# brocksam/pycollo

Measured on AMD Instinct MI355X. Metric: NLP-callback evals/sec (g + jac_g + hess), higher is better.
Workload: dtype f64; 1 GPU; hypersensitive, 1 phase, 2000 mesh sections x 6 Lobatto nodes = 10001 collocation nodes; num_x=20003, num_c=10001, nnz_jac=140003, nnz_hess=20002, tiles=167, threads_per_block=64, waves_per_tile=4, launches_per_eval=1, lds_bytes_per_workgroup=24144, launch_thread_cpu=16, pin_survived_hip_init=False

## Files before the change

__graft_entry__.py:

```python
from __future__ import annotations

import os
import subprocess
import sys

ROOT = os.path.dirname(os.path.abspath(__file__))
if ROOT not in sys.path:
    sys.path.insert(0, ROOT)

CSRC = os.path.join(ROOT, "pycollo_amd", "csrc")
LIB = os.path.join(ROOT, "pycollo_amd", "libpycollo_amd.so")


def _run(cmd):
    res = subprocess.run(cmd, capture_output=True, text=True)
    if res.returncode != 0:
        raise RuntimeError(f"{' '.join(cmd)} failed:\n{res.stdout[-2000:]}\n{res.stderr[-4000:]}")


def _stale(target, sources):
    if not os.path.exists(target):
        return True
    t = os.path.getmtime(target)
    return any(os.path.getmtime(s) > t for s in sources)


def build_library(force: bool = False) -> str:
    srcs = [os.path.join(CSRC, f) for f in ("pc_engine.hip", "pc_kkt.hip", "pc_host.hpp", "pc_ipm.hpp", "pc_kkt_cr.hpp", "pc_kkt_shape.hpp", "pc_eval_shape.hpp", "pc_eval_launch.hpp", "pc_pattern.hpp", "pc_desc.hpp", "pc_args.h", "pc_deriv.hpp", "pc_deriv_check.hpp",
                                           "pc_solution_plan.hpp", "pc_costate_plan.hpp", "pc_propagate_plan.hpp",
                                           "pc_solution_host.hpp")]
    srcs.append(os.path.join(ROOT, "include", "pycollo_amd.h"))
    if force or _stale(LIB, srcs):
        hipcc = "/opt/rocm/bin/hipcc" if os.path.exists("/opt/rocm/bin/hipcc") else "hipcc"
        _run([hipcc, "--offload-arch=gfx950", "-O2", "-ffp-contract=off", "-fPIC", "-shared", "-std=c++17", "-o", LIB + ".tmp",
              os.path.join(CSRC, "pc_engine.hip"), os.path.join(CSRC, "pc_kkt.hip")])
        os.replace(LIB + ".tmp", LIB)
    return LIB


PREBUILD = [
    ("brachistochrone", {}, (0,)), ("brachistochrone", {}, (4,)),
    ("hypersensitive", {}, (0,)), ("hypersensitive", {}, (6,)), ("hypersensitive", {}, (5,)), ("hypersensitive", {}, (4,)),
    ("hypersensitive", {}, (2,)), ("hypersensitive", {}, (8,)), ("hypersensitive", {}, (3,)),
    ("hypersensitive", {"fixed_control": 0.0}, (0,)),
    ("cart_pole", {}, (0,)), ("cart_pole", {}, (4,)), ("cart_pole", {}, (5,)),
    ("shuttle", {}, (0,)), ("shuttle", {}, (4,)), ("shuttle", {}, (5,)), ("shuttle", {}, (6,)),
    ("double_pendulum", {}, (0,)), ("double_pendulum", {}, (4,)),
    ("two_phase_transfer", {}, (0, 0)), ("two_phase_transfer", {}, (3, 4)), ("two_phase_transfer", {}, (4, 5)),
    ("two_phase_transfer", {}, (2, 2)), ("two_phase_transfer", {}, (3, 3)), ("two_phase_transfer", {}, (4, 4)),
    ("time_coupled_transfer", {}, (0, 0)), ("time_coupled_transfer", {}, (4, 4)),
    ("time_coupled_transfer", {}, (3, 3)), ("time_coupled_transfer", {}, (3, 4)),
    ("delta_iii", {}, (0, 0, 0, 0)), ("delta_iii", {}, (4, 4, 4, 4)), ("delta_iii", {}, (5, 5, 5, 5)), ("delta_iii", {}, (8, 8, 8, 8)),
    ("free_flying_robot", {}, (0,)), ("free_flying_robot", {}, (4,)), ("free_flying_robot", {}, (5,)),
    ("tumour_anti_angiogenesis", {}, (0,)), ("tumour_anti_angiogenesis", {}, (4,)), ("tumour_anti_angiogenesis", {}, (6,)),
    ("space_station", {}, (0,)), ("space_station", {}, (4,)),
    ("sliding_mass", {"num_phases": 1}, (0,)), ("sliding_mass", {"num_phases": 1}, (4,)),
    ("sliding_mass", {"num_phases": 2}, (0, 0)), ("sliding_mass", {"num_phases": 2}, (4, 4)),
    ("sliding_mass", {"num_phases": 3}, (0, 0, 0)), ("sliding_mass", {"num_phases": 3}, (4, 4, 4)),
    ("sliding_mass", {"num_phases": 4}, (0, 0, 0, 0)), ("sliding_mass", {"num_phases": 4}, (4, 4, 4, 4)),
    ("function_family", {"family": "powers"}, (0,)), ("function_family", {"family": "powers"}, (4,)),
    ("function_family", {"family": "trig"}, (0,)), ("function_family", {"family": "trig"}, (4,)),
    ("function_family", {"family": "special"}, (0,)), ("function_family", {"family": "special"}, (4,)),
    ("function_family", {"family": "kinks"}, (0,)), ("function_family", {"family": "kinks"}, (4,)),
]
PREBUILD_MIXED = [
    ("hypersensitive", {}, (4, 6)), ("cart_pole", {}, (4, 6)), ("shuttle", {}, (4, 6)), ("double_pendulum", {}, (4, 6)),
    ("two_phase_transfer", {}, (4, 6)), ("time_coupled_transfer", {}, (4, 6)), ("delta_iii", {}, (4, 6)),
    ("hypersensitive", {}, (6,)), ("two_phase_transfer", {}, (4,)), ("time_coupled_transfer", {}, (4,)), ("delta_iii", {}, (5,)),
# ... 104 lines not shown
```

pycollo_amd/codegen.py:

```python
from __future__ import annotations

import hashlib
import os
import shutil
import subprocess

import sympy as sym
from sympy.printing.c import C99CodePrinter

from .model import Model, PhaseModel, PointModel

CSRC = os.path.join(os.path.dirname(os.path.abspath(__file__)), "csrc")
CACHE = os.path.join(os.path.dirname(os.path.abspath(__file__)), "_cache")
ARCH = "gfx950"


class _Printer(C99CodePrinter):

    def _print_Pow(self, expr):
        base, exp = expr.base, expr.exp
        b = self.parenthesize(base, 200)
        if exp.is_Integer:
            n = int(exp)
            if n == 0:
# ... 285 lines not shown
    if heavy_cap is None:
        heavy_cap = _heavy_cap_enabled()
    heavy_any = any(is_heavy(pm) for pm in model.phases)
    parts = [f"// generated by pycollo_amd.codegen for model '{model.name}' digest {model.digest} -- do not edit",
             '#include "pc_kernels.hpp"',
             '#include "pc_solution.hpp"',
             "",
             POWI_PRELUDE,
             "namespace gen {"]
    for pm in model.phases:
        parts.append(_phase_struct(pm, model))
    parts.append(_point_struct(model.point))
    parts.append("}  // namespace gen\n")
    parts.append("namespace gen {")
    parts.append("struct Tail {   // finishes one evaluation: cross-tile sums of every phase and the endpoint block")
    parts.append("  // RES: block 0 of a resident-tail bulk launch (values of other workgroups arrive as granules)")
    parts.append("  template <bool RES = false, bool BIG = false>")
    parts.append("  __device__ static __forceinline__ void run(const PcTailArgs& a, const PcTailLead* ld = nullptr, int arg_off = 0,")
    parts.append("                                             int tb = 0, int ntb = 1) {")
    parts.append("    extern __shared__ double pc_tail_smem[];")
    parts.append("    const pc::TailLds L = pc::tail_lds<Point>(a, pc_tail_smem);")
    first = model.phases[0].index
    parts.append("    if constexpr (RES) {")
    parts.append("      pc::KernargWarm warm;")
    parts.append("      warm.issue<(int)sizeof(PcTailArgs)>(arg_off);   // every line of the tail's argument block, at once")
    parts.append("      pc::tail_point_load<Point, true>(a, L);")
    parts.append("      pc::tail_begin(a, L);")
    parts.append("      warm.settle();")
    parts.append("      pc::tail_point_eval<Point>(a, L, tb, ntb);   // the endpoint rows are out before the first tile's sums arrive")
    parts.append("      if (tb > 0) { pc::tail_point_publish<Point>(a, L, tb, ntb); return; }   // helper block: its parts only")
    for pm in model.phases:
        parts.append(f"      pc::tail_phase<Phase{pm.index}, true>(a, {pm.index}, L);")
    parts.append("      pc::tail_point_collect<Point>(a, L, ntb);")
    parts.append("      pc::tail_point_apply<Point, true>(a, L);")
    parts.append("      pc::tail_end(a, L);")
    parts.append("    } else {")
    parts.append(f"      pc::TailPhaseRegs<Phase{first}> r0;   // the first phase's loads go out before anything else")
    parts.append(f"      pc::tail_phase_issue<Phase{first}, false, BIG>(a, {first}, r0, ld);")
    parts.append("      __builtin_amdgcn_sched_barrier(0);")
    parts.append("      pc::tail_point_load<Point, false>(a, L);")
    parts.append("      pc::tail_begin(a, L);")
    parts.append("      pc::tail_point_eval<Point>(a, L);")
    parts.append(f"      pc::tail_phase_finish<Phase{first}>(a, {first}, r0, L);")
    for pm in model.phases[1:]:
        parts.append(f"      pc::tail_phase<Phase{pm.index}, false, BIG>(a, {pm.index}, L);")
    parts.append("      pc::tail_point_apply<Point, false>(a, L);")
    parts.append("      pc::tail_end(a, L);")
    parts.append("    }")
    parts.append("  }")
    parts.append("};")
    parts.append("}  // namespace gen\n")
    occ = _occupancy_attr()
    lead_sig = ('const double* xz, const double* lamd, const double* qa, const double* sec_h, int N, int K, '
                'int tile_begin, int n_blocks, int wa, int wb')
    parts.append("#ifndef PC_PART\n#define PC_PART -1\n#endif")
    parts.append("#if PC_PART <= 0")
    for pm in model.phases:
        hv = _heavy_attr(is_heavy(pm), heavy_cap)
        parts.append(f'extern "C" __global__ void __launch_bounds__(256) {occ}{hv}pc_bulk_p{pm.index}({lead_sig}, PcPhaseArgs a) {{')
        if mixed[pm.index] and len(model.phases) == 1:
            parts.append('  const PcPhaseArgs& ka = pc::kernarg_phase_args();   // (a itself is not named: see there)')
            parts.append('  const int blk = pc::xcd_major((int)blockIdx.x, n_blocks);')
            parts.append(f'  pc::bulk_mix<gen::Phase{pm.index}, false, 0, 0>({seq(pm)}, ka.tile_rec + blk, ka, false, 0, blk);')
        else:
            parts.append('  const PcLead ld{xz, lamd, qa, sec_h, N, K, tile_begin, n_blocks, wa, wb};')
            parts.append(f'  pc::bulk<gen::Phase{pm.index}, {int(orders[pm.index])}>(a, false, 0, -1, &ld);')
        parts.append('}')
    parts.append("#endif")
    if len(model.phases) == 1:
        pm = model.phases[0]
# ... 320 lines not shown
```

pycollo_amd/csrc/pc_kernels.hpp:

```cpp
#pragma once

#include <hip/hip_runtime.h>
#include <type_traits>
#include <utility>

#include "pc_args.h"

namespace pc {

template <int I>
using ic = std::integral_constant<int, I>;

template <int B, int E, class F>
__device__ __forceinline__ void static_for(F&& f) {
  if constexpr (B < E) {
    f(ic<B>{});
    static_for<B + 1, E>(f);
  }
}

#ifndef PC_SPLIT_MIN
#define PC_SPLIT_MIN 90
#endif

// ... 374 lines not shown

#ifndef PC_XCD_SWIZZLE
#define PC_XCD_SWIZZLE 1
#endif
__device__ __forceinline__ int xcd_major(int b, int nb) {
#if PC_XCD_SWIZZLE
  constexpr int NX = 8;
  const int q = nb / NX, r = nb % NX, x = b % NX, j = b / NX;
  return x * q + (x < r ? x : r) + j;
#else
  (void)nb;
  return b;
#endif
}

#ifdef PC_STAMPS
#ifndef PC_STAMPS_WAVES
#define PC_STAMPS_WAVES 16384
#endif
extern "C" __device__ unsigned long long pc_stamps[PC_STAMPS_WAVES * 24];
#define PC_STAMP(i)                                                                                         \
  do {                                                                                                      \
    if ((threadIdx.x & 63) == 0 && pc_stamp_slot < PC_STAMPS_WAVES)                                         \
      pc_stamps[(size_t)pc_stamp_slot * 24 + (i)] = (i) == 9 ? __builtin_amdgcn_s_memrealtime() : __builtin_amdgcn_s_memtime(); \
  } while (0)
#else
#define PC_STAMP(i) do { } while (0)
#endif

template <class M, int UN, bool RES = false, int WN = 0, int WIDX = 0, bool MIX = false>
__device__ __forceinline__ void bulk(const PcPhaseArgs& KA, bool MULTI = false, int first_block = 0, int block = -1,
                                     const PcLead* LD = nullptr, const double* mx = nullptr, const double* mlam = nullptr,
                                     double* mc = nullptr, double* mG = nullptr, double* mH = nullptr, int mflags = 0,
                                     unsigned mepoch = 0, int r_k0 = 0, int r_nsec = 0, int r_n0 = 0, int r_nprev = 0,
                                     int r_qaprev = 0, long long r_E0 = 0, double r_wprev = 0.0) {
  using St = S<M>;
  constexpr int NY = St::NY, NZ = St::NZ, NQ = St::NQ, NP = St::NP, NS = St::NS, NT = St::NT;
  constexpr int NFN = St::NFN, NV = St::NV, NJ = St::NJ, NH = St::NH, NFS = St::NFS, NRED = St::NRED;
  constexpr bool PURE = MIX && UN > 0;
  BulkIn<St> A;
  if (LD) {
    const int wa = LD->wa, wb = LD->wb;
    A.xz = LD->xz; A.lamd = LD->lamd; A.qa = LD->qa; A.sec_h = LD->sec_h; A.N = LD->N; A.K = LD->K;
    A.tile_begin = LD->tile_begin; A.n_blocks = LD->n_blocks;
    A.flags = pc_wa_flags(wa); A.wpt = pc_wa_wpt(wa); A.block_threads = pc_wa_block_threads(wa); A.spt = pc_wa_spt(wa);
    A.qa0 = pc_wb_qa_off(wb); A.qwabs = pc_wb_qw_abs(wb);
  } else {
    A.x = MULTI ? mx : KA.x; A.lam = MULTI ? mlam : KA.lam; A.x_off = KA.x_off; A.c_off = KA.c_off; A.N = KA.N; A.K = KA.K;
    A.xz = A.x + A.x_off; A.lamd = A.lam + A.c_off; A.qa = KA.qa; A.sec_h = KA.sec_h;
    A.tile_begin = KA.tile_begin; A.spt = KA.spt; A.n_blocks = KA.n_blocks;
// ... 214 lines not shown
    goff = A.goff;
    hoff = A.hoff;
  } else {
    sc = s_tab;
    goff = reinterpret_cast<const int64_t*>(s_tab + St::NSCAL);
    hoff = goff + NFN;
  }
  const bool owns = active && (t < T || last_tile);
  double F[NFN > 0 ? NFN : 1], Jv[NJ > 0 ? NJ : 1], Hv[NH > 0 ? NH : 1], mu[NFN > 0 ? NFN : 1];
  double red[NRED > 0 ? NRED : 1];
  static_for<0, NRED>([&](auto r_) { red[decltype(r_)::value] = 0.0; });
  if (active) {
    static_for<0, NS>([&](auto l_) {
      constexpr int l = decltype(l_)::value;
      constexpr int kind = M::wk(l), idx = M::wi(l);
      v[NZ + l] = A.x[kind == 0 ? A.s_off + idx : A.x_off + (int64_t)NZ * N + (kind == 1 ? idx : NQ + idx)];
    });
  }
  double lam_p[NP > 0 ? NP : 1], lam_q[NQ > 0 ? NQ : 1];
  if (owns && wantH && hess_replica) {
    static_for<0, NP>([&](auto m_) { lam_p[decltype(m_)::value] = A.lam[A.c_path_off + (int64_t) decltype(m_)::value * N + node]; });
    static_for<0, NQ>([&](auto m_) { lam_q[decltype(m_)::value] = A.lam[A.c_int_off + decltype(m_)::value]; });
  }

  const int r_off = (UN == 0 && tid < 2 * (PC_MAX_ORDER + 1)) ? reinterpret_cast<const int32_t*>(&KA.qa_off[0])[tid] : 0;
  if (!early_aux) aux_loads();
  if constexpr (UN == 0) {
    r_qa = tid < A.qa_total ? A.qa[tid] : 0.0;
    r_qw = tid < A.qw_total ? A.qw[tid] : 0.0;
  }
  pin_second_group();
  if (!uni) {
    for (int i = tid; i <= nsec; i += TB) {
      s_s[i] = A.sec_s[kp + i];
      s_E[i] = A.sec_E[kp + i];
    }
  }
  if (UN == 0 && tid < 2 * (PC_MAX_ORDER + 1)) s_off[tid] = r_off;
  if constexpr (UN > 0) {
    if (tid < QA_N) s_qa[tid] = r_qa;
    if (tid < UN) s_qw[tid] = r_qw;
  } else {
    if (tid < A.qa_total) s_qa[tid] = r_qa;
    if (tid < A.qw_total) s_qw[tid] = r_qw;
  }
  if (tid < nsec) s_h[tid] = r_h;
// ... 197 lines not shown
      const double sr = wave_sum(red[r]);
      if (lane == 0) s_red[r * 16 + wave] = sr;
    });
    if constexpr (RES) {
      lds_barrier();
      if (tid < NRED) {
        double sr = 0.0;
        for (int ww = 0; ww < nw; ++ww) sr += s_red[tid * 16 + ww];
        publish_granules(A.gran + 2 * ((int64_t)tile * NRED + tid), A.epoch, sr);
      }
    }
  }
  };
  constexpr bool SPLIT = ((NJ + NH >= PC_SPLIT_MIN) || M::HEAVY) && St::NWT == 0;
  constexpr bool RED_EARLY = RES && NS == 0 && NRED > 0;
  double mult[NFN > 0 ? NFN : 1];
  if (active) {
    static_for<0, NFN>([&](auto r_) {
      constexpr int r = decltype(r_)::value;
      mult[r] = (r >= NY && r < NY + NP) ? mu[r] : stretch * mu[r];
    });
  }
  const int n_own = T + (last_tile ? 1 : 0);
  const bool edge0 = (node == 0), edgeN = (node == N - 1);
  constexpr int NEDGE = St::NHZZ + 2 * NZ + NS * NZ;
  auto edge_store = [&](auto site_, double* dstp, double val) {
    constexpr int site = decltype(site_)::value;
    constexpr bool f0 = M::efl(site) != 0, fN = M::efl(NEDGE + site) != 0;
    if constexpr (RES && (f0 || fN)) {
      constexpr int r0 = PC_CE(St::erank(site)), rN = PC_CE(St::erank(NEDGE + site));
      if (edge0 ? f0 : fN) {
        publish_granules(A.erec + 2 * (int64_t)(A.erec0 + (edge0 ? r0 : rN)), A.epoch, val);
        return;
      }
    }
    *dstp = val;
  };
  auto hess_second = [&]() {
    static_for<0, NZ>([&](auto rv_) {
      constexpr int rv = decltype(rv_)::value;
      constexpr int MB = PC_CE(St::hrow_count(rv));
      if constexpr (MB > 0) if (mine(PC_ITEM(St::IT_HB + rv))) {
        double vals[MB];
        static_for<0, NH>([&](auto e_) {
          constexpr int e = decltype(e_)::value;
          if constexpr (M::hr(e) == rv)
            vals[PC_CE(St::hpos(e))] = sc[St::O_VZ + rv] * sc[St::O_VZ + M::hc(e)] * Hv[e];
        });
        if (owns && (edge0 || edgeN)) {
          static_for<0, NH>([&](auto e_) {
            constexpr int e = decltype(e_)::value;
            if constexpr (M::hr(e) == rv)
              edge_store(ic<St::hzz_index(e)>{}, A.H + (edge0 ? A.hslot0 : A.hslotN)[PC_CE(St::hzz_index(e))],
                         vals[PC_CE(St::hpos(e))]);
          });
        }
        if constexpr (MB == 1) {
          if (owns && !edge0 && !edgeN) A.H[hoff[St::HO_Z + rv] + (int64_t)node] = vals[0];
        } else {
          if (owns) static_for<0, MB>([&](auto q_) { s_out[t * MB + decltype(q_)::value] = vals[decltype(q_)::value]; });
          stage_sync();
          const int lo = (n0 == 0) ? 1 : 0, hi = (last_tile ? n_own - 1 : n_own);
          if (hi > lo)
            flush_run(A.H + hoff[St::HO_Z + rv] + (int64_t)(n0 + lo) * MB, s_out + lo * MB, (hi - lo) * MB, t, TN);
          stage_sync();
        }
      }
    });
    if (owns) {
      static_for<0, NH>([&](auto e_) {
        constexpr int e = decltype(e_)::value;
        constexpr int rv = M::hr(e), cv = M::hc(e);
        if constexpr (rv >= NZ && cv < NZ && St::is_t(rv >= NZ ? rv - NZ : 0)) {
        } else if constexpr (rv >= NZ && cv < NZ) {
          if (mine(PC_ITEM(St::IT_HS + cv))) {
            double* dstp = A.H + hoff[St::HO_S + (rv - NZ) * NZ + cv] + node;
            const double val = sc[St::O_VS + rv - NZ] * sc[St::O_VZ + cv] * Hv[e];
// ... 335 lines not shown
    };
    static_for<0, NY>(defect_jacobian_of_state);
  }

  PC_STAMP(5);
  if constexpr (SPLIT) {
    second_pass();
    if constexpr (!RED_EARLY) deposit_partials();
  }
  if constexpr (NRED > 0 && !RES) {
    block_sync();
    if (tid < NRED) {
      const int nw = (TB + 63) >> 6;
      double sr = 0.0;
      for (int ww = 0; ww < nw; ++ww) sr += s_red[tid * 16 + ww];
      A.partials[(int64_t)tile * NRED + tid] = sr;
    }
  }
  PC_STAMP(7);
#ifdef PC_STAMPS
  asm volatile("s_waitcnt vmcnt(0)" ::: "memory");
#endif
  PC_STAMP(8);
}
#undef PC_ITEM

__device__ __forceinline__ const PcPhaseArgs& kernarg_phase_args() {
  typedef const __attribute__((address_space(4))) char* kseg_t;
  return *(const PcPhaseArgs*)((kseg_t)__builtin_amdgcn_kernarg_segment_ptr() + sizeof(PcLead));
}

template <class M, bool RES, int WN, int WIDX, int... ORD>
__device__ __forceinline__ void bulk_mix(std::integer_sequence<int, ORD...>, const PcTileRec* rec, const PcPhaseArgs& KA,
                                         bool MULTI, int first_block, int block, const PcLead* LD = nullptr,
                                         const double* mx = nullptr, const double* mlam = nullptr, double* mc = nullptr,
                                         double* mG = nullptr, double* mH = nullptr, int mflags = 0, unsigned mepoch = 0) {
  const int order = rec->order, k0 = rec->k0, nsec = rec->nsec, n0 = rec->n0, nprev = rec->nprev, qaprev = rec->qa_prev;
  const long long E0 = rec->E0;
  const double wprev = rec->w_prev;
  const bool done = (... || (order == ORD ? (bulk<M, ORD, RES, WN, WIDX, true>(KA, MULTI, first_block, block, LD, mx, mlam, mc, mG, mH,
                                                                              mflags, mepoch, k0, nsec, n0, nprev, qaprev, E0, wprev), true)
                                          : false));
  if (!done) bulk<M, 0, RES, WN, WIDX, true>(KA, MULTI, first_block, block, LD, mx, mlam, mc, mG, mH, mflags, mepoch);
}

struct TailLds {
  double *acc, *part, *sum, *xb, *lb, *hold, *hb;
};
template <class PT>
__device__ __forceinline__ TailLds tail_lds(const PcTailArgs& A, double* base) {
  TailLds L;
  L.acc = base;
  L.part = L.acc + A.n_tail_owned;
  L.sum = L.part + 16 * A.lds_nred;
  L.xb = L.sum + A.lds_nred;
  L.lb = L.xb + PT::NPV;
  L.hold = L.lb + PT::NB;
  L.hb = L.hold + PT::NPH;
  return L;
}
__device__ __forceinline__ void tail_begin(const PcTailArgs& A, const TailLds& L) {
  if (A.flags & PC_FLAG_H)
    for (int i = threadIdx.x; i < A.n_tail_owned; i += A.block_threads) L.acc[i] = 0.0;
  lds_barrier();
}
__device__ __forceinline__ void tail_end(const PcTailArgs& A, const TailLds& L) {
  lds_barrier();
  if (A.flags & PC_FLAG_H)
    for (int i = threadIdx.x; i < A.n_tail_owned; i += A.block_threads) A.H[A.tail_owned[i]] = L.acc[i];
}
struct KernargWarm {
  unsigned acc = 0;
  template <int BYTES>
  __device__ __forceinline__ void issue(int byte_off) {
    typedef const __attribute__((address_space(4))) unsigned* kp;
    kp p = (kp)((const __attribute__((address_space(4))) char*)__builtin_amdgcn_kernarg_segment_ptr() + byte_off);
#pragma unroll
    for (int i = 0; i < BYTES / 64; ++i) acc ^= p[16 * i];
  }
  __device__ __forceinline__ void settle() const { asm volatile("" ::"s"(acc)); }
};
__device__ __forceinline__ bool spin_again(unsigned& spins, const PcTailArgs& A, unsigned code) {
  __builtin_amdgcn_s_sleep(2);
  if (++spins < (unsigned)PC_SPIN_LIMIT) return true;
  if (A.timeout) __hip_atomic_store(A.timeout, code, __ATOMIC_RELAXED, __HIP_MEMORY_SCOPE_SYSTEM);
  return false;
}

template <class M>
struct TailPhaseRegs {
  using St = S<M>;
  double xt[2], vt[2], rt[2];
  double xq[St::NQ > 0 ? St::NQ : 1], wi[St::NQ > 0 ? St::NQ : 1], vq[St::NQ > 0 ? St::NQ : 1], rq[St::NQ > 0 ? St::NQ : 1];
  double vs[St::NS > 0 ? St::NS : 1], acc[4][St::NRED > 0 ? St::NRED : 1];
};
template <class M, bool RES = false, bool BIG = false>
__device__ __forceinline__ void tail_phase_issue(const PcTailArgs& A, int ip, TailPhaseRegs<M>& R, const PcTailLead* L = nullptr) {
  using St = S<M>;
  constexpr int NZ = St::NZ, NQ = St::NQ, NS = St::NS, NT = St::NT, NRED = St::NRED;
  if constexpr (NRED > 0) {
    const PcTailPhase& P = A.ph[ip];
    const int tid = threadIdx.x, TB = L ? L->block_threads : A.block_threads;
    const int NG = 256 / TB;
    const double* xv = L ? L->x : A.x;
    const double* sc = L ? L->scal0 : P.scal;
    const int N = L ? L->N0 : P.N;
    const int64_t q_off = (L ? L->x_off0 : P.x_off) + (int64_t)NZ * N, t_off = q_off + NQ;
    double (&xt)[2] = R.xt, (&vt)[2] = R.vt, (&rt)[2] = R.rt;
    auto& xq = R.xq; auto& wi = R.wi; auto& vq = R.vq; auto& rq = R.rq; auto& vs = R.vs; auto& acc = R.acc;
    xt[0] = xt[1] = vt[0] = vt[1] = rt[0] = rt[1] = 0.0;
    if (tid == 0) {
      static_for<0, NT>([&](auto j_) {
        constexpr int j = decltype(j_)::value;
        xt[j] = xv[t_off + j];
        vt[j] = sc[St::O_VT + j];
        rt[j] = sc[St::O_RT + j];
      });
      static_for<0, NQ>([&](auto m_) {
        constexpr int m = decltype(m_)::value;
        xq[m] = xv[q_off + m];
        wi[m] = sc[St::O_WI + m];
        vq[m] = sc[St::O_VQ + m];
        rq[m] = sc[St::O_RQ + m];
      });
      static_for<0, NS>([&](auto l_) { vs[decltype(l_)::value] = sc[St::O_VS + decltype(l_)::value]; });
    }
    static_for<0, 4>([&](auto g_) { static_for<0, NRED>([&](auto r_) { acc[decltype(g_)::value][decltype(r_)::value] = 0.0; }); });
    const int nt = L ? L->n_tiles0 : P.n_tiles;
    if constexpr (RES) {
      const unsigned long long* gr = P.gran;
      unsigned spins = 0;
      constexpr int SL = NRED <= 2 ? 4 : (NRED <= 4 ? 2 : 1);
      for (int b0 = 0; b0 < nt; b0 += SL * TB) {
        double val[SL][NRED];
        for (;;) {
          unsigned long long raw[SL][2 * NRED];
          static_for<0, SL>([&](auto s_) {
            constexpr int sl = decltype(s_)::value;
            const int b = b0 + tid + TB * sl;
            if (b < nt) {
              const int64_t tile_b = xcd_major(b, nt);
              static_for<0, 2 * NRED>([&](auto i_) { raw[sl][decltype(i_)::value] = load_granule(gr + 2 * tile_b * NRED + decltype(i_)::value); });
            }
          });
          bool ok = true;
          static_for<0, SL>([&](auto s_) {
            constexpr int sl = decltype(s_)::value;
            const int b = b0 + tid + TB * sl;
            if (b < nt)
              static_for<0, NRED>([&](auto r_) {
                constexpr int r = decltype(r_)::value;
                ok &= join_granules(raw[sl][2 * r], raw[sl][2 * r + 1], A.epoch, val[sl][r]);
              });
          });
          if (__all(ok)) break;
          if (!spin_again(spins, A, 1u + (unsigned)ip)) break;
        }
        const int gb = (b0 / TB) % NG;
        static_for<0, SL>([&](auto s_) {
          constexpr int sl = decltype(s_)::value;
          const int b = b0 + tid + TB * sl;
          const int g = (gb + sl) % NG;
          static_for<0, 4>([&](auto g_) {
            constexpr int gg = decltype(g_)::value;
            const bool hit = b < nt && g == gg;
            static_for<0, NRED>([&](auto r_) { acc[gg][decltype(r_)::value] += hit ? val[sl][decltype(r_)::value] : 0.0; });
          });
        });
      }
    } else {
      const double* part = L ? L->partials0 : P.partials;
      constexpr int U = BIG ? (NRED <= 4 ? 8 : 4) : 1;
      static_for<0, 4>([&](auto g_) {
        constexpr int g = decltype(g_)::value;
        if (g >= NG) return;
        for (int b0 = tid + TB * g; b0 < nt; b0 += U * 256) {
          double tmp[U][NRED];
          static_for<0, U>([&](auto u_) {
            constexpr int u = decltype(u_)::value;
            const int b = b0 + u * 256;
            static_for<0, NRED>([&](auto r_) {
              constexpr int r = decltype(r_)::value;
              tmp[u][r] = b < nt ? part[(int64_t)xcd_major(b, nt) * NRED + r] : 0.0;
            });
          });
          static_for<0, U>([&](auto u_) {
            constexpr int u = decltype(u_)::value;
            if (b0 + u * 256 < nt) static_for<0, NRED>([&](auto r_) { acc[g][decltype(r_)::value] += tmp[u][decltype(r_)::value]; });
          });
        }
      });
    }
  }
}
template <class M>
__device__ __forceinline__ void tail_phase_finish(const PcTailArgs& A, int ip, TailPhaseRegs<M>& R, const TailLds& L) {
  using St = S<M>;
  constexpr int NZ = St::NZ, NQ = St::NQ, NP = St::NP, NY = St::NY, NS = St::NS, NT = St::NT, NRED = St::NRED;
  if constexpr (NRED > 0) {
    double* s_part = L.part;
    double* s_sum = L.sum;
    const PcTailPhase& P = A.ph[ip];
    const int tid = threadIdx.x, TB = A.block_threads, NG = 256 / TB;
    double (&xt)[2] = R.xt, (&vt)[2] = R.vt, (&rt)[2] = R.rt;
    auto& xq = R.xq; auto& wi = R.wi; auto& vq = R.vq; auto& rq = R.rq; auto& vs = R.vs; auto& acc = R.acc;
    lds_barrier();
    static_for<0, 4>([&](auto g_) {
      constexpr int g = decltype(g_)::value;
      if (g >= NG) return;
      static_for<0, NRED>([&](auto r_) {
        constexpr int r = decltype(r_)::value;
        const double w = wave_sum(acc[g][r]);
        if ((tid & 63) == 0) s_part[r * 16 + (tid >> 6) + (TB >> 6) * g] = w;
      });
    });
    lds_barrier();
    if (tid == 0) {
      static_for<0, NRED>([&](auto r_) {
        constexpr int r = decltype(r_)::value;
        double tot = s_part[r * 16];
        for (int w = 1; w < 4; ++w) tot += s_part[r * 16 + w];
        s_sum[r] = tot;
      });
      double* hacc = L.acc;
      double t0 = P.t_fixed[0], tF = P.t_fixed[1], dst[2] = {0.0, 0.0};
      int j = 0;
      if constexpr (M::T0_FREE) {
        t0 = vt[j] * xt[j] + rt[j];
        dst[j] = -0.5 * vt[j];
        ++j;
      }
      if constexpr (M::TF_FREE) {
        tF = vt[j] * xt[j] + rt[j];
        dst[j] = 0.5 * vt[j];
      }
      const double stretch = 0.5 * (tF - t0);
      static_for<0, NQ>([&](auto m_) {
        constexpr int m = decltype(m_)::value;
        constexpr int r = NY + NP + m;
        const double Wi = wi[m];
        if (A.flags & PC_FLAG_C) {
          const double q = vq[m] * xq[m] + rq[m];
          A.c[P.c_int_off + m] = Wi * (q - stretch * s_sum[St::R_Q + m]);
        }
        if (A.flags & PC_FLAG_G) {
          int64_t o = P.gq_base[m];
          auto dgdw = [&](auto l_) -> double {
            constexpr int l = decltype(l_)::value;
            return -Wi * stretch * vs[l] * s_sum[PC_CE(St::rqs(m, l))];
          };
          static_for<0, NS>([&](auto l_) {
            constexpr int l = decltype(l_)::value;
            if constexpr (St::is_q(l) && M::wi(l) < m && PC_CE(St::dep(r, NZ + l))) A.G[o++] = dgdw(l_);
          });
          {
            double val = Wi * vq[m];
            constexpr int lq = PC_CE(St::qpar(m));
            if constexpr (lq >= 0) {
              if constexpr (PC_CE(St::dep(r, NZ + (lq >= 0 ? lq : 0)))) val += dgdw(ic<(lq >= 0 ? lq : 0)>{});
            }
            A.G[o++] = val;
          }
          static_for<0, NS>([&](auto l_) {
            constexpr int l = decltype(l_)::value;
            if constexpr (St::is_q(l) && M::wi(l) > m && PC_CE(St::dep(r, NZ + l))) A.G[o++] = dgdw(l_);
          });
          static_for<0, NT>([&](auto jt_) {
            constexpr int jt = decltype(jt_)::value;
            double val = -Wi * dst[jt] * s_sum[St::R_Q + m];
            constexpr int lt = PC_CE(St::tpar(jt));
            if constexpr (lt >= 0) {
              if constexpr (PC_CE(St::dep(r, NZ + (lt >= 0 ? lt : 0)))) val += dgdw(ic<(lt >= 0 ? lt : 0)>{});
            }
            A.G[o++] = val;
          });
          static_for<0, NS>([&](auto l_) {
            constexpr int l = decltype(l_)::value;
            if constexpr (M::wk(l) == 0 && PC_CE(St::dep(r, NZ + l))) A.G[o++] = dgdw(l_);
          });
        }
      });
      if (A.flags & PC_FLAG_H) {
        static_for<0, NS>([&](auto l_) {
          constexpr int l = decltype(l_)::value;
          if constexpr (NT > 0 && PC_CE(St::tz(NZ + l))) {
            static_for<0, NT>([&](auto jt_) {
              constexpr int jt = decltype(jt_)::value;
              constexpr double twice = (St::is_t(l) && M::wi(l) == jt) ? 2.0 : 1.0;
              hacc[P.hsum_local[jt * NS + l]] += twice * (dst[jt] * vs[l] * s_sum[PC_CE(St::rts(l))]);
            });
          }
        });
        static_for<0, St::NH>([&](auto e_) {
          constexpr int e = decltype(e_)::value;
          if constexpr (M::hc(e) >= NZ) {
            constexpr int l = M::hr(e) - NZ, l2 = M::hc(e) - NZ;
            hacc[P.hsum_local[2 * NS + l * (l + 1) / 2 + l2]] += s_sum[PC_CE(St::rss(l, l2))];
          }
        });
      }
    }
  }
}
template <class M, bool RES = false, bool BIG = false>
__device__ __forceinline__ void tail_phase(const PcTailArgs& A, int ip, const TailLds& L) {
  TailPhaseRegs<M> R;
  tail_phase_issue<M, RES, BIG>(A, ip, R);
  tail_phase_finish<M>(A, ip, R, L);
}

template <class PT, bool RES = false>
__device__ __forceinline__ void tail_point_load(const PcTailArgs& A, const TailLds& L) {
  constexpr int NPV = PT::NPV, NB = PT::NB, NPH = PT::NPH;
  const bool wantH = A.flags & PC_FLAG_H;
  const int tid = threadIdx.x, TB = A.block_threads;
  for (int i = tid; i < NPV; i += TB) L.xb[i] = A.pt_V[i] * A.x[A.pt_x[i]] + A.pt_r[i];
  for (int r = tid; r < NB; r += TB) L.lb[r] = wantH ? A.lam[A.c_end_off + r] * A.pt_W[r] : 0.0;
  if constexpr (!RES) {
    if (wantH)
      for (int e = tid; e < NPH; e += TB) L.hold[e] = A.pt_hlocal[e] < 0 ? A.H[A.pt_hslot[e]] : 0.0;
  }
}
template <class PT>
__device__ __forceinline__ void tail_point_eval(const PcTailArgs& A, const TailLds& L, int tb = 0, int ntb = 1) {
  constexpr int NPV = PT::NPV, NB = PT::NB, NGJ = PT::NGJ, NBJ = PT::NBJ, NPH = PT::NPH;
  const int tid = threadIdx.x, wave = tid >> 6, nw = (A.block_threads + 63) >> 6;
  if ((tid & 63) != 0) return;
  const double sigma = A.sigma, wJ = A.wJ;
  const bool wantH = A.flags & PC_FLAG_H;
  static_for<0, PT::NPARTS>([&](auto g_) {
    constexpr int g = decltype(g_)::value;
    if (g % ntb != tb || (g / ntb) % nw != wave) return;
    double xb[NPV > 0 ? NPV : 1], lb[NB > 0 ? NB : 1];
    static_for<0, NPV>([&](auto i_) { xb[decltype(i_)::value] = L.xb[decltype(i_)::value]; });
    static_for<0, NB>([&](auto r_) { lb[decltype(r_)::value] = L.lb[decltype(r_)::value]; });
    double Jval = 0.0, gJ[NGJ > 0 ? NGJ : 1], b[NB > 0 ? NB : 1], jb[NBJ > 0 ? NBJ : 1], hb[NPH > 0 ? NPH : 1];
    PT::template eval_part<g>(xb, sigma * wJ, lb, Jval, gJ, b, jb, hb);
    if constexpr (g == 0) {
      if (A.fobj) A.fobj[0] = wJ * Jval;
      if (A.grad_nz) {
        static_for<0, NGJ>([&](auto e_) {
          constexpr int e = decltype(e_)::value;
          A.grad_nz[e] = wJ * gJ[e] * A.pt_V[PT::gc(e)];
// ... 8 lines not shown
    if (A.flags & PC_FLAG_G)
      static_for<0, NBJ>([&](auto e_) {
        constexpr int e = decltype(e_)::value;
        if constexpr (PT::part_jb(e) == g) A.G[A.g_end_base + e] = A.pt_W[PT::br(e)] * jb[e] * A.pt_V[PT::bc(e)];
      });
    if (wantH)
      static_for<0, NPH>([&](auto e_) {
        constexpr int e = decltype(e_)::value;
        if constexpr (PT::part_hb(e) == g) L.hb[e] = hb[e] * A.pt_V[PT::phr(e)] * A.pt_V[PT::phc(e)];
      });
  });
}
template <class PT>
__device__ __forceinline__ void tail_point_publish(const PcTailArgs& A, const TailLds& L, int tb, int ntb) {
  constexpr int NPH = PT::NPH;
  lds_barrier();
  if constexpr (NPH > 0) {
    if (!(A.flags & PC_FLAG_H)) return;
    for (int e = threadIdx.x; e < NPH; e += A.block_threads)
      if (PT::part_hb(e) % ntb == tb) publish_granules(A.hb_gran + 2 * e, A.epoch, L.hb[e]);
  }
}
template <class PT>
__device__ __forceinline__ void tail_point_collect(const PcTailArgs& A, const TailLds& L, int ntb) {
  constexpr int NPH = PT::NPH;
  if constexpr (NPH > 0) {
    if (ntb <= 1 || !(A.flags & PC_FLAG_H)) return;
    unsigned spins = 0;
    for (int e0 = 0; e0 < NPH; e0 += A.block_threads) {
      const int e = e0 + threadIdx.x;
      const bool mine = e < NPH && PT::part_hb(e) % ntb != 0;
      double v = 0.0;
      for (;;) {
        bool ok = true;
        if (mine) {
          const unsigned long long lo = load_granule(A.hb_gran + 2 * e), hi = load_granule(A.hb_gran + 2 * e + 1);
          ok = join_granules(lo, hi, A.epoch, v);
        }
        if (__all(ok)) break;
        if (!spin_again(spins, A, 200u)) break;
      }
      if (mine) L.hb[e] = v;
    }
  }
}

template <class PT, bool RES = false>
__device__ __forceinline__ void tail_point_apply(const PcTailArgs& A, const TailLds& L) {
  constexpr int NPH = PT::NPH;
  lds_barrier();
  if (!(A.flags & PC_FLAG_H)) return;
  const int tid = threadIdx.x, TB = A.block_threads;
  if constexpr (NPH > 0) {
    for (int e = tid; e < NPH; e += TB) {
      const int hl = A.pt_hlocal[e];
      if (hl >= 0) L.acc[hl] += L.hb[e];
      else if constexpr (!RES) A.H[A.pt_hslot[e]] = L.hold[e] + L.hb[e];
    }
  }
  if constexpr (RES) {
    unsigned spins = 0;
    for (int r0 = 0; r0 < A.n_rec; r0 += TB) {
      const int r = r0 + tid;
      const int64_t slot = r < A.n_rec ? A.rec_slot[r] : -1;
      const bool live = slot >= 0;
      double cur = 0.0;
      for (;;) {
        bool ok = true;
        if (live) {
          const unsigned long long* g = A.erec + 2 * (int64_t)r;
          const unsigned long long lo = load_granule(g), hi = load_granule(g + 1);
          ok = join_granules(lo, hi, A.epoch, cur);
        }
        if (__all(ok)) break;
        if (!spin_again(spins, A, 100u)) break;
      }
      if (live) {
        const int term = A.rec_term[r];
        if constexpr (NPH > 0) A.H[slot] = term >= 0 ? cur + L.hb[term] : cur;
        else A.H[slot] = cur;
      }
    }
  }
}

}
```

Measured before the change: 236,900 evals/s.

## Prefetch tail and edge Hessian slot tables early to hide load latency

Moves the tail kernel's index-table loads (owned slots, hlocal/hslot, record slots/terms, phase hsum_local, t_fixed, gq_base) and kernel argument pointers into registers at the start, so the final stores no longer wait on dependent global loads. It also loads the edge Hessian slots for the first and last nodes early in the main tile kernel. Adds timing-stamp macros compiled only under PC_STAMPS, and prebuilds two more configurations. The cost is extra register pressure and more code complexity across the tail path.

```diff
diff --git a/__graft_entry__.py b/__graft_entry__.py
--- a/__graft_entry__.py
+++ b/__graft_entry__.py
@@ -44,6 +44,7 @@
     ("hypersensitive", {}, (2,)), ("hypersensitive", {}, (8,)), ("hypersensitive", {}, (3,)),
     ("hypersensitive", {"fixed_control": 0.0}, (0,)),
     ("cart_pole", {}, (0,)), ("cart_pole", {}, (4,)), ("cart_pole", {}, (5,)),
+    ("cart_pole", {}, (3,)), ("space_station", {}, (3,)),
     ("shuttle", {}, (0,)), ("shuttle", {}, (4,)), ("shuttle", {}, (5,)), ("shuttle", {}, (6,)),
     ("double_pendulum", {}, (0,)), ("double_pendulum", {}, (4,)),
     ("two_phase_transfer", {}, (0, 0)), ("two_phase_transfer", {}, (3, 4)), ("two_phase_transfer", {}, (4, 5)),
diff --git a/pycollo_amd/codegen.py b/pycollo_amd/codegen.py
--- a/pycollo_amd/codegen.py
+++ b/pycollo_amd/codegen.py
@@ -331,30 +331,41 @@
     parts.append("    const pc::TailLds L = pc::tail_lds<Point>(a, pc_tail_smem);")
     first = model.phases[0].index
     parts.append("    if constexpr (RES) {")
+    parts.append("      PC_TAIL_STAMP(0);")
+    parts.append("      PC_TAIL_STAMP(9);")
     parts.append("      pc::KernargWarm warm;")
     parts.append("      warm.issue<(int)sizeof(PcTailArgs)>(arg_off);   // every line of the tail's argument block, at once")
-    parts.append("      pc::tail_point_load<Point, true>(a, L);")
+    parts.append("      const pc::TailEarly E = pc::tail_early<Point, true>(a);   // table values of the tail's END, requested now")
+    parts.append("      pc::tail_point_load<Point, true>(a, L, E);")
     parts.append("      pc::tail_begin(a, L);")
     parts.append("      warm.settle();")
+    parts.append("      pc::tail_early_settle(E);")
     parts.append("      pc::tail_point_eval<Point>(a, L, tb, ntb);   // the endpoint rows are out before the first tile's sums arrive")
     parts.append("      if (tb > 0) { pc::tail_point_publish<Point>(a, L, tb, ntb); return; }   // helper block: its parts only")
     for pm in model.phases:
-        parts.append(f"      pc::tail_phase<Phase{pm.index}, true>(a, {pm.index}, L);")
-    parts.append("      pc::tail_point_collect<Point>(a, L, ntb);")
-    parts.append("      pc::tail_point_apply<Point, true>(a, L);")
-    parts.append("      pc::tail_end(a, L);")
+        parts.append(f"      pc::tail_phase<Phase{pm.index}, true>(a, {pm.index}, L, E);")
+    parts.append("      pc::tail_point_collect<Point>(a, L, E, ntb);")
+    parts.append("      pc::tail_point_apply<Point, true>(a, L, E);")
+    parts.append("      pc::tail_end(L, E);")
+    parts.append("      PC_TAIL_STAMP(21);   // last store issued")
+    parts.append("#ifdef PC_STAMPS")
+    parts.append('      asm volatile("s_waitcnt vmcnt(0)" ::: "memory");')
+    parts.append("      PC_TAIL_STAMP(22);")
+    parts.append("#endif")
     parts.append("    } else {")
     parts.append(f"      pc::TailPhaseRegs<Phase{first}> r0;   // the first phase's loads go out before anything else")
     parts.append(f"      pc::tail_phase_issue<Phase{first}, false, BIG>(a, {first}, r0, ld);")
     parts.append("      __builtin_amdgcn_sched_barrier(0);")
-    parts.append("      pc::tail_point_load<Point, false>(a, L);")
+    parts.append("      const pc::TailEarly E = pc::tail_early<Point, false>(a);")
+    parts.append("      pc::tail_point_load<Point, false>(a, L, E);")
     parts.append("      pc::tail_begin(a, L);")
+    parts.append("      pc::tail_early_settle(E);")
     parts.append("      pc::tail_point_eval<Point>(a, L);")
-    parts.append(f"      pc::tail_phase_finish<Phase{first}>(a, {first}, r0, L);")
+    parts.append(f"      pc::tail_phase_finish<Phase{first}>(r0, L, E);")
     for pm in model.phases[1:]:
-        parts.append(f"      pc::tail_phase<Phase{pm.index}, false, BIG>(a, {pm.index}, L);")
-    parts.append("      pc::tail_point_apply<Point, false>(a, L);")
-    parts.append("      pc::tail_end(a, L);")
+        parts.append(f"      pc::tail_phase<Phase{pm.index}, false, BIG>(a, {pm.index}, L, E);")
+    parts.append("      pc::tail_point_apply<Point, false>(a, L, E);")
+    parts.append("      pc::tail_end(L, E);")
     parts.append("    }")
     parts.append("  }")
     parts.append("};")
diff --git a/pycollo_amd/csrc/pc_kernels.hpp b/pycollo_amd/csrc/pc_kernels.hpp
--- a/pycollo_amd/csrc/pc_kernels.hpp
+++ b/pycollo_amd/csrc/pc_kernels.hpp
@@ -420,10 +420,16 @@
 #define PC_STAMP(i)                                                                                         \
   do {                                                                                                      \
     if ((threadIdx.x & 63) == 0 && pc_stamp_slot < PC_STAMPS_WAVES)                                         \
-      pc_stamps[(size_t)pc_stamp_slot * 24 + (i)] = (i) == 9 ? __builtin_amdgcn_s_memrealtime() : __builtin_amdgcn_s_memtime(); \
+      ::pc::pc_stamps[(size_t)pc_stamp_slot * 24 + (i)] = ((i) == 9 || (i) >= 20) ? __builtin_amdgcn_s_memrealtime() : __builtin_amdgcn_s_memtime(); \
+  } while (0)
+#define PC_TAIL_STAMP(i)                                                                                    \
+  do {                                                                                                      \
+    const int pc_stamp_slot = (int)blockIdx.x * (int)(blockDim.x >> 6) + (int)(threadIdx.x >> 6);           \
+    PC_STAMP(i);                                                                                            \
   } while (0)
 #else
 #define PC_STAMP(i) do { } while (0)
+#define PC_TAIL_STAMP(i) do { } while (0)
 #endif
 
 template <class M, int UN, bool RES = false, int WN = 0, int WIDX = 0, bool MIX = false>
@@ -684,6 +690,24 @@
     static_for<0, NP>([&](auto m_) { lam_p[decltype(m_)::value] = A.lam[A.c_path_off + (int64_t) decltype(m_)::value * N + node]; });
     static_for<0, NQ>([&](auto m_) { lam_q[decltype(m_)::value] = A.lam[A.c_int_off + decltype(m_)::value]; });
   }
+#ifndef PC_EDGE_SLOTS_MAX
+#define PC_EDGE_SLOTS_MAX 8
+#endif
+  const bool edge0 = (node == 0), edgeN = (node == N - 1);
+  constexpr bool EDGE_EARLY = St::NHZZ > 0 && St::NHZZ <= PC_EDGE_SLOTS_MAX;
+  int64_t eslot[EDGE_EARLY ? St::NHZZ : 1];
+  if constexpr (EDGE_EARLY) {
+    static_for<0, St::NHZZ>([&](auto i_) { eslot[decltype(i_)::value] = 0; });
+    if (owns && wantH && hess_replica && (edge0 || edgeN)) {
+      const int64_t* hs = edge0 ? A.hslot0 : A.hslotN;
+      static_for<0, NH>([&](auto e_) {
+        constexpr int e = decltype(e_)::value;
+        if constexpr (M::hr(e) < NZ) {
+          if (mine(PC_ITEM(St::IT_HB + M::hr(e)))) eslot[PC_CE(St::hzz_index(e))] = hs[PC_CE(St::hzz_index(e))];
+        }
+      });
+    }
+  }
 
   const int r_off = (UN == 0 && tid < 2 * (PC_MAX_ORDER + 1)) ? reinterpret_cast<const int32_t*>(&KA.qa_off[0])[tid] : 0;
   if (!early_aux) aux_loads();
@@ -927,7 +951,6 @@
     });
   }
   const int n_own = T + (last_tile ? 1 : 0);
-  const bool edge0 = (node == 0), edgeN = (node == N - 1);
   constexpr int NEDGE = St::NHZZ + 2 * NZ + NS * NZ;
   auto edge_store = [&](auto site_, double* dstp, double val) {
     constexpr int site = decltype(site_)::value;
@@ -955,9 +978,12 @@
         if (owns && (edge0 || edgeN)) {
           static_for<0, NH>([&](auto e_) {
             constexpr int e = decltype(e_)::value;
-            if constexpr (M::hr(e) == rv)
-              edge_store(ic<St::hzz_index(e)>{}, A.H + (edge0 ? A.hslot0 : A.hslotN)[PC_CE(St::hzz_index(e))],
-                         vals[PC_CE(St::hpos(e))]);
+            if constexpr (M::hr(e) == rv) {
+              int64_t slot;
+              if constexpr (EDGE_EARLY) slot = eslot[PC_CE(St::hzz_index(e))];
+              else slot = (edge0 ? A.hslot0 : A.hslotN)[PC_CE(St::hzz_index(e))];
+              edge_store(ic<St::hzz_index(e)>{}, A.H + slot, vals[PC_CE(St::hpos(e))]);
+            }
           });
         }
         if constexpr (MB == 1) {
@@ -1339,6 +1365,7 @@
   asm volatile("s_waitcnt vmcnt(0)" ::: "memory");
 #endif
   PC_STAMP(8);
+  PC_STAMP(22);
 }
 #undef PC_ITEM
 
@@ -1381,10 +1408,59 @@
     for (int i = threadIdx.x; i < A.n_tail_owned; i += A.block_threads) L.acc[i] = 0.0;
   lds_barrier();
 }
-__device__ __forceinline__ void tail_end(const PcTailArgs& A, const TailLds& L) {
+struct TailEarly {
+  int64_t owned = 0;
+  int64_t hslot = 0;
+  int64_t rec_slot = -1;
+  int rec_term = -1;
+  int hlocal = -1;
+  double *c, *G, *H;
+  const int64_t *tail_owned, *rec_slot_tab;
+  const int32_t* rec_term_tab;
+  const unsigned long long* erec;
+  unsigned* timeout;
+  int n_tail_owned, flags, block_threads, n_rec;
+  unsigned epoch;
+};
+template <class PT, bool RES>
+__device__ __forceinline__ TailEarly tail_early(const PcTailArgs& A) {
+  TailEarly E;
+  const int tid = threadIdx.x;
+  if (A.flags & PC_FLAG_H) {
+    if (tid < A.n_tail_owned) E.owned = A.tail_owned[tid];
+    if constexpr (PT::NPH > 0) {
+      if (tid < PT::NPH) {
+        E.hlocal = A.pt_hlocal[tid];
+        if constexpr (!RES) E.hslot = A.pt_hslot[tid];
+      }
+    }
+    if constexpr (RES) {
+      if (tid < A.n_rec) {
+        E.rec_slot = A.rec_slot[tid];
+        E.rec_term = A.rec_term[tid];
+      }
+    }
+  }
+  E.c = A.c; E.G = A.G; E.H = A.H; E.tail_owned = A.tail_owned; E.n_tail_owned = A.n_tail_owned; E.flags = A.flags;
+  E.block_threads = A.block_threads;
+  E.erec = A.erec; E.rec_slot_tab = A.rec_slot; E.rec_term_tab = A.rec_term; E.n_rec = RES ? A.n_rec : 0; E.epoch = A.epoch;
+  E.timeout = A.timeout;
+  PinAcc pin;
+  pin(E.c); pin(E.G); pin(E.H); pin(E.tail_owned); pin(E.n_tail_owned); pin(E.flags); pin(E.block_threads);
+  if constexpr (RES) { pin(E.erec); pin(E.rec_slot_tab); pin(E.rec_term_tab); pin(E.n_rec); pin((int)E.epoch); pin(E.timeout); }
+  pin.done();
+  return E;
+}
+__device__ __forceinline__ void tail_early_settle(const TailEarly& E) {
+  asm volatile("" ::"v"(E.owned), "v"(E.hslot), "v"(E.rec_slot), "v"(E.rec_term), "v"(E.hlocal));
+}
+__device__ __forceinline__ void tail_end(const TailLds& L, const TailEarly& E) {
   lds_barrier();
-  if (A.flags & PC_FLAG_H)
-    for (int i = threadIdx.x; i < A.n_tail_owned; i += A.block_threads) A.H[A.tail_owned[i]] = L.acc[i];
+  if (E.flags & PC_FLAG_H) {
+    const int tid = threadIdx.x;
+    if (tid < E.n_tail_owned) E.H[E.owned] = L.acc[tid];
+    for (int i = tid + E.block_threads; i < E.n_tail_owned; i += E.block_threads) E.H[E.tail_owned[i]] = L.acc[i];
+  }
 }
 struct KernargWarm {
   unsigned acc = 0;
@@ -1397,10 +1473,10 @@
   }
   __device__ __forceinline__ void settle() const { asm volatile("" ::"s"(acc)); }
 };
-__device__ __forceinline__ bool spin_again(unsigned& spins, const PcTailArgs& A, unsigned code) {
+__device__ __forceinline__ bool spin_again(unsigned& spins, unsigned* timeout, unsigned code) {
   __builtin_amdgcn_s_sleep(2);
   if (++spins < (unsigned)PC_SPIN_LIMIT) return true;
-  if (A.timeout) __hip_atomic_store(A.timeout, code, __ATOMIC_RELAXED, __HIP_MEMORY_SCOPE_SYSTEM);
+  if (timeout) __hip_atomic_store(timeout, code, __ATOMIC_RELAXED, __HIP_MEMORY_SCOPE_SYSTEM);
   return false;
 }
 
@@ -1410,6 +1486,9 @@
   double xt[2], vt[2], rt[2];
   double xq[St::NQ > 0 ? St::NQ : 1], wi[St::NQ > 0 ? St::NQ : 1], vq[St::NQ > 0 ? St::NQ : 1], rq[St::NQ > 0 ? St::NQ : 1];
   double vs[St::NS > 0 ? St::NS : 1], acc[4][St::NRED > 0 ? St::NRED : 1];
+  int hl[St::NS > 0 ? 2 * St::NS + St::NS * (St::NS + 1) / 2 : 1];
+  double t_fixed[2];
+  int64_t c_int_off, gq_base[St::NQ > 0 ? St::NQ : 1];
 };
 template <class M, bool RES = false, bool BIG = false>
 __device__ __forceinline__ void tail_phase_issue(const PcTailArgs& A, int ip, TailPhaseRegs<M>& R, const PcTailLead* L = nullptr) {
@@ -1442,11 +1521,34 @@
       });
       static_for<0, NS>([&](auto l_) { vs[decltype(l_)::value] = sc[St::O_VS + decltype(l_)::value]; });
     }
+    auto phase_tables = [&]() {
+      if (tid == 0 && ((L ? L->flags : A.flags) & PC_FLAG_H)) {
+        static_for<0, NS>([&](auto l_) {
+          constexpr int l = decltype(l_)::value;
+          if constexpr (NT > 0 && PC_CE(St::tz(NZ + l)))
+            static_for<0, NT>([&](auto jt_) { R.hl[decltype(jt_)::value * NS + l] = P.hsum_local[decltype(jt_)::value * NS + l]; });
+        });
+        static_for<0, St::NH>([&](auto e_) {
+          constexpr int e = decltype(e_)::value;
+          if constexpr (M::hc(e) >= NZ) {
+            constexpr int k = 2 * NS + (M::hr(e) - NZ) * (M::hr(e) - NZ + 1) / 2 + (M::hc(e) - NZ);
+            R.hl[k] = P.hsum_local[k];
+          }
+        });
+      }
+      R.t_fixed[0] = P.t_fixed[0]; R.t_fixed[1] = P.t_fixed[1]; R.c_int_off = P.c_int_off;
+      static_for<0, NQ>([&](auto m_) { R.gq_base[decltype(m_)::value] = P.gq_base[decltype(m_)::value]; });
+      PinAcc pin;
+      pin(R.t_fixed[0]); pin(R.t_fixed[1]); pin(R.c_int_off);
+      static_for<0, NQ>([&](auto m_) { pin(R.gq_base[decltype(m_)::value]); });
+      pin.done();
+    };
     static_for<0, 4>([&](auto g_) { static_for<0, NRED>([&](auto r_) { acc[decltype(g_)::value][decltype(r_)::value] = 0.0; }); });
     const int nt = L ? L->n_tiles0 : P.n_tiles;
     if constexpr (RES) {
       const unsigned long long* gr = P.gran;
       unsigned spins = 0;
+      phase_tables();
       constexpr int SL = NRED <= 2 ? 4 : (NRED <= 4 ? 2 : 1);
       for (int b0 = 0; b0 < nt; b0 += SL * TB) {
         double val[SL][NRED];
@@ -1471,7 +1573,7 @@
               });
           });
           if (__all(ok)) break;
-          if (!spin_again(spins, A, 1u + (unsigned)ip)) break;
+          if (!spin_again(spins, A.timeout, 1u + (unsigned)ip)) break;
         }
         const int gb = (b0 / TB) % NG;
         static_for<0, SL>([&](auto s_) {
@@ -1485,6 +1587,7 @@
           });
         });
       }
+      PC_TAIL_STAMP(20);
     } else {
       const double* part = L ? L->partials0 : P.partials;
       constexpr int U = BIG ? (NRED <= 4 ? 8 : 4) : 1;
@@ -1507,18 +1610,18 @@
           });
         }
       });
+      phase_tables();
     }
   }
 }
 template <class M>
-__device__ __forceinline__ void tail_phase_finish(const PcTailArgs& A, int ip, TailPhaseRegs<M>& R, const TailLds& L) {
+__device__ __forceinline__ void tail_phase_finish(TailPhaseRegs<M>& R, const TailLds& L, const TailEarly& E) {
   using St = S<M>;
   constexpr int NZ = St::NZ, NQ = St::NQ, NP = St::NP, NY = St::NY, NS = St::NS, NT = St::NT, NRED = St::NRED;
   if constexpr (NRED > 0) {
     double* s_part = L.part;
     double* s_sum = L.sum;
-    const PcTailPhase& P = A.ph[ip];
-    const int tid = threadIdx.x, TB = A.block_threads, NG = 256 / TB;
+    const int tid = threadIdx.x, TB = E.block_threads, NG = 256 / TB;
     double (&xt)[2] = R.xt, (&vt)[2] = R.vt, (&rt)[2] = R.rt;
     auto& xq = R.xq; auto& wi = R.wi; auto& vq = R.vq; auto& rq = R.rq; auto& vs = R.vs; auto& acc = R.acc;
     lds_barrier();
@@ -1533,6 +1636,24 @@
     });
     lds_barrier();
     if (tid == 0) {
+      auto arrived = [](double v) { asm volatile("" ::"v"(v)); };
+      static_for<0, NT>([&](auto j_) { arrived(xt[decltype(j_)::value]); arrived(vt[decltype(j_)::value]); arrived(rt[decltype(j_)::value]); });
+      static_for<0, NQ>([&](auto m_) {
+        constexpr int m = decltype(m_)::value;
+        arrived(xq[m]); arrived(wi[m]); arrived(vq[m]); arrived(rq[m]);
+      });
+      static_for<0, NS>([&](auto l_) { arrived(vs[decltype(l_)::value]); });
+      if (E.flags & PC_FLAG_H) {
+        auto arrived_i = [](int v) { asm volatile("" ::"v"(v)); };
+        static_for<0, NS>([&](auto l_) {
+          constexpr int l = decltype(l_)::value;
+          if constexpr (NT > 0 && PC_CE(St::tz(NZ + l))) static_for<0, NT>([&](auto jt_) { arrived_i(R.hl[decltype(jt_)::value * NS + l]); });
+        });
+        static_for<0, St::NH>([&](auto e_) {
+          constexpr int e = decltype(e_)::value;
+          if constexpr (M::hc(e) >= NZ) arrived_i(R.hl[2 * NS + (M::hr(e) - NZ) * (M::hr(e) - NZ + 1) / 2 + (M::hc(e) - NZ)]);
+        });
+      }
       static_for<0, NRED>([&](auto r_) {
         constexpr int r = decltype(r_)::value;
         double tot = s_part[r * 16];
@@ -1540,7 +1661,7 @@
         s_sum[r] = tot;
       });
       double* hacc = L.acc;
-      double t0 = P.t_fixed[0], tF = P.t_fixed[1], dst[2] = {0.0, 0.0};
+      double t0 = R.t_fixed[0], tF = R.t_fixed[1], dst[2] = {0.0, 0.0};
       int j = 0;
       if constexpr (M::T0_FREE) {
         t0 = vt[j] * xt[j] + rt[j];
@@ -1556,19 +1677,19 @@
         constexpr int m = decltype(m_)::value;
         constexpr int r = NY + NP + m;
         const double Wi = wi[m];
-        if (A.flags & PC_FLAG_C) {
+        if (E.flags & PC_FLAG_C) {
           const double q = vq[m] * xq[m] + rq[m];
-          A.c[P.c_int_off + m] = Wi * (q - stretch * s_sum[St::R_Q + m]);
+          E.c[R.c_int_off + m] = Wi * (q - stretch * s_sum[St::R_Q + m]);
         }
-        if (A.flags & PC_FLAG_G) {
-          int64_t o = P.gq_base[m];
+        if (E.flags & PC_FLAG_G) {
+          int64_t o = R.gq_base[m];
           auto dgdw = [&](auto l_) -> double {
             constexpr int l = decltype(l_)::value;
             return -Wi * stretch * vs[l] * s_sum[PC_CE(St::rqs(m, l))];
           };
           static_for<0, NS>([&](auto l_) {
             constexpr int l = decltype(l_)::value;
-            if constexpr (St::is_q(l) && M::wi(l) < m && PC_CE(St::dep(r, NZ + l))) A.G[o++] = dgdw(l_);
+            if constexpr (St::is_q(l) && M::wi(l) < m && PC_CE(St::dep(r, NZ + l))) E.G[o++] = dgdw(l_);
           });
           {
             double val = Wi * vq[m];
@@ -1576,11 +1697,11 @@
             if constexpr (lq >= 0) {
               if constexpr (PC_CE(St::dep(r, NZ + (lq >= 0 ? lq : 0)))) val += dgdw(ic<(lq >= 0 ? lq : 0)>{});
             }
-            A.G[o++] = val;
+            E.G[o++] = val;
           }
           static_for<0, NS>([&](auto l_) {
             constexpr int l = decltype(l_)::value;
-            if constexpr (St::is_q(l) && M::wi(l) > m && PC_CE(St::dep(r, NZ + l))) A.G[o++] = dgdw(l_);
+            if constexpr (St::is_q(l) && M::wi(l) > m && PC_CE(St::dep(r, NZ + l))) E.G[o++] = dgdw(l_);
           });
           static_for<0, NT>([&](auto jt_) {
             constexpr int jt = decltype(jt_)::value;
@@ -1589,22 +1710,22 @@
             if constexpr (lt >= 0) {
               if constexpr (PC_CE(St::dep(r, NZ + (lt >= 0 ? lt : 0)))) val += dgdw(ic<(lt >= 0 ? lt : 0)>{});
             }
-            A.G[o++] = val;
+            E.G[o++] = val;
           });
           static_for<0, NS>([&](auto l_) {
             constexpr int l = decltype(l_)::value;
-            if constexpr (M::wk(l) == 0 && PC_CE(St::dep(r, NZ + l))) A.G[o++] = dgdw(l_);
+            if constexpr (M::wk(l) == 0 && PC_CE(St::dep(r, NZ + l))) E.G[o++] = dgdw(l_);
           });
         }
       });
-      if (A.flags & PC_FLAG_H) {
+      if (E.flags & PC_FLAG_H) {
         static_for<0, NS>([&](auto l_) {
           constexpr int l = decltype(l_)::value;
           if constexpr (NT > 0 && PC_CE(St::tz(NZ + l))) {
             static_for<0, NT>([&](auto jt_) {
               constexpr int jt = decltype(jt_)::value;
               constexpr double twice = (St::is_t(l) && M::wi(l) == jt) ? 2.0 : 1.0;
-              hacc[P.hsum_local[jt * NS + l]] += twice * (dst[jt] * vs[l] * s_sum[PC_CE(St::rts(l))]);
+              hacc[R.hl[jt * NS + l]] += twice * (dst[jt] * vs[l] * s_sum[PC_CE(St::rts(l))]);
             });
           }
         });
@@ -1612,7 +1733,7 @@
           constexpr int e = decltype(e_)::value;
           if constexpr (M::hc(e) >= NZ) {
             constexpr int l = M::hr(e) - NZ, l2 = M::hc(e) - NZ;
-            hacc[P.hsum_local[2 * NS + l * (l + 1) / 2 + l2]] += s_sum[PC_CE(St::rss(l, l2))];
+            hacc[R.hl[2 * NS + l * (l + 1) / 2 + l2]] += s_sum[PC_CE(St::rss(l, l2))];
           }
         });
       }
@@ -1620,14 +1741,14 @@
   }
 }
 template <class M, bool RES = false, bool BIG = false>
-__device__ __forceinline__ void tail_phase(const PcTailArgs& A, int ip, const TailLds& L) {
+__device__ __forceinline__ void tail_phase(const PcTailArgs& A, int ip, const TailLds& L, const TailEarly& E) {
   TailPhaseRegs<M> R;
   tail_phase_issue<M, RES, BIG>(A, ip, R);
-  tail_phase_finish<M>(A, ip, R, L);
+  tail_phase_finish<M>(R, L, E);
 }
 
 template <class PT, bool RES = false>
-__device__ __forceinline__ void tail_point_load(const PcTailArgs& A, const TailLds& L) {
+__device__ __forceinline__ void tail_point_load(const PcTailArgs& A, const TailLds& L, const TailEarly& E) {
   constexpr int NPV = PT::NPV, NB = PT::NB, NPH = PT::NPH;
   const bool wantH = A.flags & PC_FLAG_H;
   const int tid = threadIdx.x, TB = A.block_threads;
@@ -1635,7 +1756,10 @@
   for (int r = tid; r < NB; r += TB) L.lb[r] = wantH ? A.lam[A.c_end_off + r] * A.pt_W[r] : 0.0;
   if constexpr (!RES) {
     if (wantH)
-      for (int e = tid; e < NPH; e += TB) L.hold[e] = A.pt_hlocal[e] < 0 ? A.H[A.pt_hslot[e]] : 0.0;
+      for (int e = tid; e < NPH; e += TB) {
+        const bool first = e == tid;
+        L.hold[e] = (first ? E.hlocal : A.pt_hlocal[e]) < 0 ? A.H[first ? E.hslot : A.pt_hslot[e]] : 0.0;
+      }
   }
 }
 template <class PT>
@@ -1690,10 +1814,10 @@
   }
 }
 template <class PT>
-__device__ __forceinline__ void tail_point_collect(const PcTailArgs& A, const TailLds& L, int ntb) {
+__device__ __forceinline__ void tail_point_collect(const PcTailArgs& A, const TailLds& L, const TailEarly& E, int ntb) {
   constexpr int NPH = PT::NPH;
   if constexpr (NPH > 0) {
-    if (ntb <= 1 || !(A.flags & PC_FLAG_H)) return;
+    if (ntb <= 1 || !(E.flags & PC_FLAG_H)) return;
     unsigned spins = 0;
     for (int e0 = 0; e0 < NPH; e0 += A.block_threads) {
       const int e = e0 + threadIdx.x;
@@ -1706,7 +1830,7 @@
           ok = join_granules(lo, hi, A.epoch, v);
         }
         if (__all(ok)) break;
-        if (!spin_again(spins, A, 200u)) break;
+        if (!spin_again(spins, A.timeout, 200u)) break;
       }
       if (mine) L.hb[e] = v;
     }
@@ -1714,42 +1838,43 @@
 }
 
 template <class PT, bool RES = false>
-__device__ __forceinline__ void tail_point_apply(const PcTailArgs& A, const TailLds& L) {
+__device__ __forceinline__ void tail_point_apply(const PcTailArgs& A, const TailLds& L, const TailEarly& E) {
   constexpr int NPH = PT::NPH;
   lds_barrier();
-  if (!(A.flags & PC_FLAG_H)) return;
-  const int tid = threadIdx.x, TB = A.block_threads;
+  if (!(E.flags & PC_FLAG_H)) return;
+  const int tid = threadIdx.x, TB = E.block_threads;
   if constexpr (NPH > 0) {
     for (int e = tid; e < NPH; e += TB) {
-      const int hl = A.pt_hlocal[e];
+      const bool first = e == tid;
+      const int hl = first ? E.hlocal : A.pt_hlocal[e];
       if (hl >= 0) L.acc[hl] += L.hb[e];
-      else if constexpr (!RES) A.H[A.pt_hslot[e]] = L.hold[e] + L.hb[e];
+      else if constexpr (!RES) E.H[first ? E.hslot : A.pt_hslot[e]] = L.hold[e] + L.hb[e];
     }
   }
   if constexpr (RES) {
     unsigned spins = 0;
-    for (int r0 = 0; r0 < A.n_rec; r0 += TB) {
+    for (int r0 = 0; r0 < E.n_rec; r0 += TB) {
       const int r = r0 + tid;
-      const int64_t slot = r < A.n_rec ? A.rec_slot[r] : -1;
+      const int64_t slot = r0 == 0 ? E.rec_slot : (r < E.n_rec ? E.rec_slot_tab[r] : -1);
       const bool live = slot >= 0;
       double cur = 0.0;
       for (;;) {
         bool ok = true;
         if (live) {
-          const unsigned long long* g = A.erec + 2 * (int64_t)r;
+          const unsigned long long* g = E.erec + 2 * (int64_t)r;
           const unsigned long long lo = load_granule(g), hi = load_granule(g + 1);
-          ok = join_granules(lo, hi, A.epoch, cur);
+          ok = join_granules(lo, hi, E.epoch, cur);
         }
         if (__all(ok)) break;
-        if (!spin_again(spins, A, 100u)) break;
+        if (!spin_again(spins, E.timeout, 100u)) break;
       }
       if (live) {
-        const int term = A.rec_term[r];
-        if constexpr (NPH > 0) A.H[slot] = term >= 0 ? cur + L.hb[term] : cur;
-        else A.H[slot] = cur;
-      }
-    }
-  }
-}
-
-}
+        const int term = r0 == 0 ? E.rec_term : E.rec_term_tab[r];
+        if constexpr (NPH > 0) E.H[slot] = term >= 0 ? cur + L.hb[term] : cur;
+        else E.H[slot] = cur;
+      }
+    }
+  }
+}
+
+}
```

After: 236,800 evals/s. About the same (-0.1%).
